# liruiluo/VLA-Adapter

Measured on AMD Instinct MI355X. Metric: fine-tune samples/sec (224px img + 32-tok prompt), adapter-only, fwd+bwd+AdamW, higher is better.
Workload: dtype bf16

## Files before the change

### vla_adapter_amd/csrc/gemm256.hip

```cpp
#include <type_traits>
#include "gemm_epilogue.h"
#include "gemm_params.h"

namespace {

constexpr int BK = 64;
constexpr int HT = 16384;
constexpr int LDS_BYTES = 8 * HT;
constexpr int STG = 8192;

#define VLA_MMA_QUADRANT(Q, FB, FA)                                                                                                   \
  do {                                                                                                                                \
    if constexpr (F8) {                                                                                                               \
      _Pragma("unroll") for (int ni = 0; ni < 2; ++ni)                                                                                \
        _Pragma("unroll") for (int mi = 0; mi < 4; ++mi)                                                                              \
          Q[ni][mi] = __builtin_amdgcn_mfma_scale_f32_16x16x128_f8f6f4(cat8(FB[ni][0], FB[ni][1]), cat8(FA[mi][0], FA[mi][1]), Q[ni][mi], \
                                                                       0, 0, 0, 0x7f7f7f7f, 0, 0x7f7f7f7f);                            \
    } else {                                                                                                                          \
      _Pragma("unroll") for (int s = 0; s < 2; ++s)                                                                                   \
        _Pragma("unroll") for (int ni = 0; ni < 2; ++ni)                                                                              \
          _Pragma("unroll") for (int mi = 0; mi < 4; ++mi)                                                                            \
            Q[ni][mi] = __builtin_amdgcn_mfma_f32_16x16x32_bf16(FB[ni][s], FA[mi][s], Q[ni][mi], 0, 0, 0);                            \
    }                                                                                                                                 \
  } while (0)

template <int EPI, bool F8 = false, bool RES = true, bool R2 = false, bool EXT = false>
__global__ __launch_bounds__(512) void gemm256_kernel(GemmP p) {
  extern __shared__ __attribute__((aligned(16))) char smem[];
  constexpr int EB = F8 ? 1 : 2;
  constexpr bool HAS_RES = EPI == 0 && RES;
  constexpr bool PRE = EPI != 2;
  const int tid = threadIdx.x, lane = tid & 63;
  const int wid = __builtin_amdgcn_readfirstlane(tid >> 6);
  const int wr = wid >> 2, wc = wid & 3;

  const int G = gridDim.x, bid = blockIdx.x;
  const int total = p.ntiles * p.batch;
  const int q8 = total >> 3, r8 = total & 7;
  const int xcd = bid & 7;
  auto rstart = [&](int x) { return x < r8 ? x * (q8 + 1) : r8 * (q8 + 1) + (x - r8) * q8; };
  int vt = bid;
  constexpr int GM = 6;
  int m0, n0, z;
  const char* Ab; const char* Bb;
  unsigned oa[2][2], ob[2][2];
  unsigned oa2[EXT ? 2 : 1][2], ob2[EXT ? 2 : 1][2];
  auto setup = [&](int swz) {
    int sl = lane;
    asm volatile("" : "+v"(sl));
    const int kc = ((sl & 7) ^ ((sl >> 3) & 7)) * 16;
    const int lrow = sl >> 3;
    int gA = p.gA;
    asm volatile("" : "+s"(gA));
    int ntl = p.ntiles;
    asm volatile("" : "+s"(ntl));
    z = swz / ntl;
    const int tl = swz - z * ntl;
    int br = ntl / p.tiles_n, bc = p.tiles_n;
    asm volatile("" : "+s"(br), "+s"(bc));
    const int pgb = GM * bc;
    const int grp = tl / pgb, rem = tl - grp * pgb;
    const int gmr = min(GM, br - grp * GM);
    m0 = (grp * GM + rem % gmr) * 256;
    n0 = (rem / gmr) * 256;
    Ab = reinterpret_cast<const char*>(p.A) + (long long)z * p.sA * EB;
    Bb = reinterpret_cast<const char*>(p.B) + (long long)z * p.sB * EB;
#pragma unroll
    for (int h = 0; h < 2; ++h)
#pragma unroll
      for (int j = 0; j < 2; ++j) {
        const int ra = min(m0 + wr * 128 + h * 64 + (wid & 3) * 16 + j * 8 + lrow, p.M - 1);
        oa[h][j] = (unsigned)(grouped_row(ra, gA, p.sgA, p.lda) * EB + kc);
        const int rb = min(n0 + (wid >> 1) * 64 + h * 32 + (wid & 1) * 16 + j * 8 + lrow, p.N - 1);
        ob[h][j] = (unsigned)((long long)rb * p.ldb * EB + kc);
        if constexpr (EXT) {
          oa2[h][j] = (unsigned)((long long)ra * p.lda2 * 2 + kc);
          ob2[h][j] = (unsigned)((long long)rb * p.ldb2 * 2 + kc);
        }
      }
  };
  const unsigned wdst = (unsigned)(size_t)((__attribute__((address_space(3))) char*)smem) + wid * 2048;
  auto stage_a = [&](int slot, int h, int k0) {
    if (EXT && k0 >= p.K) {
      const char* b2 = reinterpret_cast<const char*>(p.A2) + (k0 - p.K) * 2;
      glds16s(b2, oa2[EXT ? h : 0][0], wdst + slot * HT);
      glds16s(b2, oa2[EXT ? h : 0][1], wdst + slot * HT + 1024);
      return;
    }
    glds16s(Ab + k0 * 2, oa[h][0], wdst + slot * HT);
    glds16s(Ab + k0 * 2, oa[h][1], wdst + slot * HT + 1024);
  };
  auto stage_b = [&](int slot, int h, int k0) {
    if (EXT && k0 >= p.K) {
      const char* b2 = reinterpret_cast<const char*>(p.B2) + (k0 - p.K) * 2;
      glds16s(b2, ob2[EXT ? h : 0][0], wdst + slot * HT);
      glds16s(b2, ob2[EXT ? h : 0][1], wdst + slot * HT + 1024);
      return;
    }
    glds16s(Bb + k0 * 2, ob[h][0], wdst + slot * HT);
    glds16s(Bb + k0 * 2, ob[h][1], wdst + slot * HT + 1024);
  };
  auto stage_k0 = [&](int buf) {
    stage_b(buf * 4 + 0, 0, 0); stage_a(buf * 4 + 1, 0, 0); stage_b(buf * 4 + 2, 1, 0); stage_a(buf * 4 + 3, 1, 0);
  };
  uint2 braw[4];
  auto bias_vec = [&]() {
    const bf16_t* bias = (EPI != 2 && p.bias) ? p.bias + (long long)z * p.sBias : nullptr;
    return bias != nullptr && (((size_t)bias & 7) == 0) && p.N >= 4;
  };
  auto fetch_bias = [&](bool bvec) {
    int sl = lane;
    asm volatile("" : "+v"(sl));
    const int lq = sl >> 4;
    long long dist = bvec ? (long long)((uintptr_t)(p.bias + (long long)z * p.sBias) - (uintptr_t)p.B) : 0;
    int lim = bvec ? p.N : 0;
    asm volatile("" : "+s"(dist), "+s"(lim));
    const bf16_t* src = reinterpret_cast<const bf16_t*>(reinterpret_cast<const char*>(p.B) + dist);
#pragma unroll
    for (int t4 = 0; t4 < 4; ++t4) {
      const int n = n0 + wc * 64 + t4 * 16 + lq * 4;
      braw[t4] = *reinterpret_cast<const uint2*>(src + (n + 3 < lim ? n : 0));
    }
  };

  const int nt = p.K / (F8 ? 2 * BK : BK) + (EXT ? p.K2 / BK : 0);

  const int aoff = wr * 64 * 128, boff = wc * 32 * 128;

  int cur = rstart(xcd) + (bid >> 3);
  if (p.stagger > 0 && (total - 1 - bid) / G + 1 < (total + G - 1) / G) {
    for (int i = 0; i < p.stagger; ++i) __builtin_amdgcn_s_sleep(16);
  }
  setup(cur);
  stage_k0(0);
  int d = 0;

  for (;;) {
    vt += G;
    const int nxt = vt < total ? rstart(vt & 7) + (vt >> 3) : -1;
    asm volatile("" : "+s"(cur));
    setup(cur);
    const bool bvec = bias_vec();
    if (nt > 1) {
      const int sn = (d ^ 1) * 4;
      stage_b(sn + 0, 0, BK); stage_a(sn + 1, 0, BK); stage_b(sn + 2, 1, BK);
    }
    fetch_bias(bvec);
    if (nt > 1) asm volatile("s_waitcnt vmcnt(10)" ::: "memory");
    else asm volatile("s_waitcnt vmcnt(4)" ::: "memory");
    VLA_BARRIER();
    int fl = lane;
    asm volatile("" : "+v"(fl));
    const int fo0 = (fl & 15) * 128 + ((((F8 ? 2 * (fl >> 4) : 0 + (fl >> 4))) ^ (fl & 7)) << 4);
    const int fo1 = (fl & 15) * 128 + ((((F8 ? 2 * (fl >> 4) + 1 : 4 + (fl >> 4))) ^ (fl & 7)) << 4);
    if (wr == 1) VLA_BARRIER();

    f32x4 acc[2][2][2][4];
#pragma unroll
    for (int a = 0; a < 2; ++a)
#pragma unroll
      for (int b = 0; b < 2; ++b)
#pragma unroll
        for (int c = 0; c < 2; ++c)
#pragma unroll
          for (int e = 0; e < 4; ++e) acc[a][b][c][e] = f32x4{0.f, 0.f, 0.f, 0.f};

    bf16x8 fa[4][2], fb0[2][2], fb1[2][2];
    for (int t = 0; t < nt; ++t) {
      const char* kb = smem + d * 4 * HT;
      const int so = d * 4, sn = (d ^ 1) * 4;
      {
        const char* sb = kb + 0 * HT + boff;
#pragma unroll
        for (int ni = 0; ni < 2; ++ni) {
          fb0[ni][0] = *reinterpret_cast<const bf16x8*>(sb + ni * 2048 + fo0);
          fb0[ni][1] = *reinterpret_cast<const bf16x8*>(sb + ni * 2048 + fo1);
        }
        const char* sa = kb + 1 * HT + aoff;
#pragma unroll
        for (int mi = 0; mi < 4; ++mi) {
          fa[mi][0] = *reinterpret_cast<const bf16x8*>(sa + mi * 2048 + fo0);
          fa[mi][1] = *reinterpret_cast<const bf16x8*>(sa + mi * 2048 + fo1);
        }
        const char* sb1 = kb + 2 * HT + boff;
#pragma unroll
        for (int ni = 0; ni < 2; ++ni) {
          fb1[ni][0] = *reinterpret_cast<const bf16x8*>(sb1 + ni * 2048 + fo0);
          fb1[ni][1] = *reinterpret_cast<const bf16x8*>(sb1 + ni * 2048 + fo1);
        }
        __builtin_amdgcn_sched_barrier(0);
        if (t + 1 < nt) {
          stage_a(sn + 3, 1, (t + 1) * BK);
          if (t > 0) asm volatile("s_waitcnt vmcnt(8)" ::: "memory");
        } else if (t > 0) {
          asm volatile("s_waitcnt vmcnt(0)" ::: "memory");
        }
        asm volatile("s_waitcnt lgkmcnt(0)" ::: "memory");
        VLA_BARRIER();
        __builtin_amdgcn_s_setprio(1);
        VLA_MMA_QUADRANT(acc[0][0], fb0, fa);
        VLA_MMA_QUADRANT(acc[0][1], fb1, fa);
        __builtin_amdgcn_s_setprio(0);
        VLA_BARRIER();
      }
      {
        const char* sa = kb + 3 * HT + aoff;
#pragma unroll
        for (int mi = 0; mi < 4; ++mi) {
          fa[mi][0] = *reinterpret_cast<const bf16x8*>(sa + mi * 2048 + fo0);
          fa[mi][1] = *reinterpret_cast<const bf16x8*>(sa + mi * 2048 + fo1);
        }
        __builtin_amdgcn_sched_barrier(0);
        if (t + 2 < nt) {
          stage_b(so + 0, 0, (t + 2) * BK); stage_a(so + 1, 0, (t + 2) * BK); stage_b(so + 2, 1, (t + 2) * BK);
          asm volatile("s_waitcnt vmcnt(8)" ::: "memory");
        } else if (t + 1 < nt) {
          asm volatile("s_waitcnt vmcnt(2)" ::: "memory");
        } else {
          asm volatile("s_waitcnt vmcnt(0)" ::: "memory");
        }
        asm volatile("s_waitcnt lgkmcnt(0)" ::: "memory");
        VLA_BARRIER();
        __builtin_amdgcn_s_setprio(1);
        VLA_MMA_QUADRANT(acc[1][1], fb1, fa);
        VLA_MMA_QUADRANT(acc[1][0], fb0, fa);
        __builtin_amdgcn_s_setprio(0);
        VLA_BARRIER();
      }
      d ^= 1;
    }
    if (wr == 0) VLA_BARRIER();
    asm volatile("s_waitcnt lgkmcnt(0)" ::: "memory");

    const int em0 = m0, en0 = n0, ez = z;
    int el = lane;
    asm volatile("" : "+v"(el));
    const int lq = el >> 4, lr = el & 15;
    int gR = p.gR, gC = p.gC, res_mod = p.res_mod, c_live_mod = p.c_live_mod;
    asm volatile("" : "+s"(gR), "+s"(gC), "+s"(res_mod), "+s"(c_live_mod));
    const bf16_t* bias = (EPI != 2 && p.bias) ? p.bias + (long long)ez * p.sBias : nullptr;
    const int wn0 = en0 + wc * 64;
    if constexpr (F8) {
#pragma unroll
      for (int t4 = 0; t4 < 4; ++t4) {
        float sbv[4];
#pragma unroll
        for (int j = 0; j < 4; ++j) sbv[j] = p.scaleB[min(wn0 + t4 * 16 + lq * 4 + j, p.N - 1)];
#pragma unroll
        for (int mh = 0; mh < 2; ++mh)
#pragma unroll
          for (int mi = 0; mi < 4; ++mi) {
            const float sav = p.scaleA[min(em0 + wr * 128 + mh * 64 + mi * 16 + lr, p.M - 1)];
#pragma unroll
            for (int j = 0; j < 4; ++j) acc[mh][t4 >> 1][t4 & 1][mi][j] *= sav * sbv[j];
          }
      }
    }
    float bv[4][4];
    int ebvec = __builtin_amdgcn_readfirstlane(bias_vec() ? 1 : 0);
    asm volatile("" : "+s"(ebvec));
#pragma unroll
    for (int t4 = 0; t4 < 4; ++t4) {
      const int n = wn0 + t4 * 16 + lq * 4;
      const bool ok = ebvec != 0 && n + 3 < p.N;
      bv[t4][0] = ok ? bf_lo(braw[t4].x) : 0.f; bv[t4][1] = ok ? bf_hi(braw[t4].x) : 0.f;
      bv[t4][2] = ok ? bf_lo(braw[t4].y) : 0.f; bv[t4][3] = ok ? bf_hi(braw[t4].y) : 0.f;
      if (bias && !ok) {
#pragma unroll
        for (int j = 0; j < 4; ++j)
          if (n + j < p.N) bv[t4][j] = bf2f(bias[n + j]);
      }
    }
    bf16_t* Cb = p.C + (long long)ez * p.sC;
    const bf16_t* Rb = (HAS_RES && p.R) ? p.R + (long long)ez * p.sR : nullptr;
    const bool vec_ok = ((p.ldc & 7) == 0) && (!Rb || (p.ldr & 7) == 0);
    const bool plain_rows = (res_mod | gR | gC | c_live_mod) == 0;
    const bool live_rows = EPI == 1 && (res_mod | gR | gC) == 0 && c_live_mod >= 64;
    bool skip[2], inside[2], fastm[2];
#pragma unroll
    for (int mh = 0; mh < 2; ++mh) {
      const int wm0 = em0 + wr * 128 + mh * 64;
      skip[mh] = wm0 >= p.M || wn0 >= p.N;
      inside[mh] = wm0 + 64 <= p.M && wn0 + 64 <= p.N;
      fastm[mh] = EPI != 2 && (plain_rows || live_rows) && vec_ok && inside[mh] && !skip[mh];
    }
    u32x4 rv[2][8];
    int fres0 = 0, fres1 = 0;
    const char* rsrc = nullptr;
    if constexpr (HAS_RES) {
      long long rdist = Rb ? (long long)((uintptr_t)Rb - (uintptr_t)p.B) : 0;
      fres0 = __builtin_amdgcn_readfirstlane((fastm[0] && Rb) ? 1 : 0);
      fres1 = __builtin_amdgcn_readfirstlane((fastm[1] && Rb) ? 1 : 0);
      asm volatile("" : "+s"(rdist), "+s"(fres0), "+s"(fres1));
      rsrc = reinterpret_cast<const char*>(p.B) + rdist;
    }
    auto load_res = [&](int mh, int it0, int it1) {
#pragma unroll
      for (int it = it0; it < it1; ++it) {
        const long long off = ((long long)(em0 + wr * 128 + mh * 64 + it * 8 + (el >> 3)) * p.ldr + wn0 + (el & 7) * 8) * 2;
        rv[mh][it] = *reinterpret_cast<const u32x4*>(rsrc + ((mh == 0 ? fres0 : fres1) ? off : 0));
      }
    };
    auto drop_res = [&](int mh) {
      asm volatile("" ::"v"(rv[mh][0]), "v"(rv[mh][1]), "v"(rv[mh][2]), "v"(rv[mh][3]), "v"(rv[mh][4]), "v"(rv[mh][5]), "v"(rv[mh][6]),
                   "v"(rv[mh][7]));
    };
    if (PRE && nxt >= 0) { setup(nxt); stage_k0(d); }
    char* const reg = PRE ? smem + (d ^ 1) * 4 * HT + wid * STG : smem + wid * STG;
    if constexpr (HAS_RES) load_res(0, 0, 4);

    if constexpr (EPI == 2) {
#pragma unroll
      for (int mh = 0; mh < 2; ++mh) {
        const int wm0 = em0 + wr * 128 + mh * 64;
        auto A4 = [&](int t4, int mi) -> f32x4& { return acc[mh][t4 >> 1][t4 & 1][mi]; };
          const bf16_t* GU = p.R + (long long)ez * p.sR;
          bf16_t* Cb = p.C + (long long)ez * p.sC;
          constexpr int ROWB = 2 * 64 * 2 + 16;
          char* reg2 = smem + wid * (32 * ROWB);
#pragma unroll
          for (int half = 0; half < 2; ++half) {
#pragma unroll
            for (int mq = 0; mq < 2; ++mq) {
              const int mi = 2 * half + mq;
              const int m = min(wm0 + mi * 16 + lr, p.M - 1);
#pragma unroll
              for (int t4 = 0; t4 < 4; ++t4) {
                const int hc = wn0 + t4 * 16 + lq * 4;
                const long long go = grouped_row(m, gR, p.sgR, p.ldr) + (hc >> 4) * 32 + (hc & 15);
                const bool ok = hc + 3 < p.N;
                const uint2 gv = ok ? *reinterpret_cast<const uint2*>(GU + go) : uint2{0, 0};
                const uint2 uv = ok ? *reinterpret_cast<const uint2*>(GU + go + 16) : uint2{0, 0};
                float gg[4], uu[4], dg[4], du[4];
                unpack4(gv, gg);
                unpack4(uv, uu);
#pragma unroll
                for (int j = 0; j < 4; ++j) swiglu_bwd(rbf(A4(t4, mi)[j] * p.alpha), gg[j], uu[j], dg[j], du[j]);
                char* rowp = reg2 + (mq * 16 + lr) * ROWB + (t4 * 32 + lq * 4) * 2;
                *reinterpret_cast<uint2*>(rowp) = pack4(dg);
                *reinterpret_cast<uint2*>(rowp + 32) = pack4(du);
              }
            }
#pragma unroll
            for (int it = 0; it < 8; ++it) {
              const int row = it * 4 + (el >> 4), ch = el & 15;
              const int m = wm0 + half * 32 + row, n2 = 2 * wn0 + ch * 8;
              if (m < p.M && n2 + 8 <= 2 * p.N)
                *reinterpret_cast<uint4*>(Cb + (long long)m * p.ldc + n2) = *reinterpret_cast<const uint4*>(reg2 + row * ROWB + ch * 16);
            }
          }
      }
    } else {
      uint2 pk[2][4][4];
      uint2 hp[2][2][4];
      if constexpr (EPI == 1) {
        const bool plain = bias == nullptr && p.alpha == 1.f;
#pragma unroll
        for (int mh = 0; mh < 2; ++mh)
#pragma unroll
          for (int pr = 0; pr < 2; ++pr)
#pragma unroll
            for (int mi = 0; mi < 4; ++mi) {
              f32x4 ga = acc[mh][pr][0][mi], ua = acc[mh][pr][1][mi];
              if (!plain) {
#pragma unroll
                for (int j = 0; j < 4; ++j) { ga[j] = epi_linear(ga[j], p.alpha, bv[2 * pr][j]); ua[j] = epi_linear(ua[j], p.alpha, bv[2 * pr + 1][j]); }
              }
              const uint2 gp = pack4(ga), up = pack4(ua);
              float g[4], u[4], h[4];
              unpack4(gp, g);
              unpack4(up, u);
#pragma unroll
              for (int j = 0; j < 4; ++j) h[j] = swiglu_h(g[j], u[j]);
              pk[mh][2 * pr][mi] = gp;
              pk[mh][2 * pr + 1][mi] = up;
              hp[mh][pr][mi] = pack4(h);
            }
      } else {
        auto phase_a = [&](auto fn, auto post_t) {
          constexpr bool POST = decltype(post_t)::value;
          const float alpha = p.alpha;
#pragma unroll
          for (int mh = 0; mh < 2; ++mh)
#pragma unroll
            for (int t4 = 0; t4 < 4; ++t4)
#pragma unroll
              for (int mi = 0; mi < 4; ++mi) {
                const f32x4 a = acc[mh][t4 >> 1][t4 & 1][mi];
                float x[4];
#pragma unroll
                for (int j = 0; j < 4; ++j) {
                  x[j] = fn(epi_linear<POST>(a[j], alpha, bv[t4][j]));
                }
                pk[mh][t4][mi] = uint2{pack2(x[0], x[1]), pack2(x[2], x[3])};
              }
        };
        auto phase_a_rope = [&]() {
          const float alpha = p.alpha;
#pragma unroll
          for (int mh = 0; mh < 2; ++mh)
#pragma unroll
            for (int mi = 0; mi < 4; ++mi) {
              const int pos = min(em0 + wr * 128 + mh * 64 + mi * 16 + lr, p.M - 1) % p.rope_T;
#pragma unroll
              for (int ni = 0; ni < 2; ++ni) {
                const int d = ni * 16 + lq * 4;
                const f32x4 c = *reinterpret_cast<const f32x4*>(p.rope_cos + (long long)pos * 32 + d);
                const f32x4 sn = *reinterpret_cast<const f32x4*>(p.rope_sin + (long long)pos * 32 + d);
                const f32x4 xa = acc[mh][0][ni][mi], xb = acc[mh][1][ni][mi];
                float ya[4], yb[4];
#pragma unroll
                for (int j = 0; j < 4; ++j) {
                  const float a = rbf(epi_linear(xa[j], alpha, bv[ni][j])), b = rbf(epi_linear(xb[j], alpha, bv[ni + 2][j]));
                  ya[j] = rope_rot_a(a, b, c[j], sn[j]);
                  yb[j] = rope_rot_b(a, b, c[j], sn[j]);
                }
                pk[mh][ni][mi] = uint2{pack2(ya[0], ya[1]), pack2(ya[2], ya[3])};
                pk[mh][ni + 2][mi] = uint2{pack2(yb[0], yb[1]), pack2(yb[2], yb[3])};
              }
              __builtin_amdgcn_sched_barrier(0);
            }
        };
        auto phase_a_rope2 = [&](auto post_t) {
          constexpr bool POST = decltype(post_t)::value;
          const float alpha = p.alpha;
#pragma unroll
          for (int mh = 0; mh < 2; ++mh)
#pragma unroll
            for (int mi = 0; mi < 4; ++mi) {
              const int pos = min(em0 + wr * 128 + mh * 64 + mi * 16 + lr, p.M - 1) % p.rope_T;
#pragma unroll
              for (int t4 = 0; t4 < 4; ++t4) {
                const int d = (wn0 + t4 * 16 + lq * 4) % p.rope_dh;
                const f32x4 c = *reinterpret_cast<const f32x4*>(p.rope_cos + (long long)pos * p.rope_dh + d);
                const f32x4 sn = *reinterpret_cast<const f32x4*>(p.rope_sin + (long long)pos * p.rope_dh + d);
                const f32x4 a = acc[mh][t4 >> 1][t4 & 1][mi];
                float x[4];
#pragma unroll
                for (int j = 0; j < 4; ++j) {
                  x[j] = rbf(epi_linear<POST>(a[j], alpha, bv[t4][j]));
                }
                const float y0 = rope_rot_a(x[0], x[1], c[0], sn[0]), y1 = rope_rot_b(x[0], x[1], c[1], sn[1]);
                const float y2 = rope_rot_a(x[2], x[3], c[2], sn[2]), y3 = rope_rot_b(x[2], x[3], c[3], sn[3]);
                pk[mh][t4][mi] = uint2{pack2(y0, y1), pack2(y2, y3)};
                if (t4 & 1) __builtin_amdgcn_sched_barrier(0);
              }
            }
        };
        if (p.rope_mode == 1 && wn0 < p.rope_cols) phase_a_rope();
        else if (R2 && p.rope_mode == 2 && wn0 < p.rope_cols) {
          if (p.bias_post) phase_a_rope2(std::true_type{});
          else phase_a_rope2(std::false_type{});
        } else if (p.bias_post) phase_a(ActNone{}, std::true_type{});
        else if (p.act == VLA_ACT_GELU) phase_a(ActGelu{}, std::false_type{});
        else if (p.act == VLA_ACT_RELU) phase_a(ActRelu{}, std::false_type{});
        else if (p.act == VLA_ACT_GELU_TANH) phase_a(ActGeluTanh{}, std::false_type{});
        else phase_a(ActNone{}, std::false_type{});
      }
#pragma unroll
      for (int mh = 0; mh < 2; ++mh)
#pragma unroll
        for (int t4 = 0; t4 < 4; ++t4)
          asm volatile("" : "+v"(pk[mh][t4][0].x), "+v"(pk[mh][t4][0].y), "+v"(pk[mh][t4][1].x), "+v"(pk[mh][t4][1].y),
                            "+v"(pk[mh][t4][2].x), "+v"(pk[mh][t4][2].y), "+v"(pk[mh][t4][3].x), "+v"(pk[mh][t4][3].y));
      asm volatile("" : "+v"(el));
      if constexpr (HAS_RES) { load_res(0, 4, 8); load_res(1, 0, 8); }
#pragma unroll
      for (int mh = 0; mh < 2; ++mh) {
        const int wm0 = em0 + wr * 128 + mh * 64;
        if (skip[mh]) {
          if constexpr (HAS_RES) drop_res(mh);
          continue;
        }
        if constexpr (EPI == 1) {
          bf16_t* C2 = p.C2 + (long long)ez * p.sC2;
          constexpr int HSTR = 32 * 2 + 16;
#pragma unroll
          for (int pr = 0; pr < 2; ++pr)
#pragma unroll
            for (int mi = 0; mi < 4; ++mi)
              *reinterpret_cast<uint2*>(reg + (mi * 16 + lr) * HSTR + (pr * 16 + lq * 4) * 2) = hp[mh][pr][mi];
          const bool hvec = ((p.ldc2 & 7) == 0) && (((size_t)C2 & 15) == 0);
          uint4 hv[4];
#pragma unroll
          for (int it = 0; it < 4; ++it) hv[it] = *reinterpret_cast<const uint4*>(reg + (it * 16 + (el >> 2)) * HSTR + (el & 3) * 16);
          __builtin_amdgcn_sched_barrier(0);
#pragma unroll
          for (int it = 0; it < 4; ++it) {
            const int row = it * 16 + (el >> 2), ch = el & 3;
            const int m = wm0 + row, hc = (wn0 >> 1) + ch * 8;
            const uint4 v = hv[it];
            if (hvec && inside[mh]) {
              *reinterpret_cast<uint4*>(C2 + (long long)m * p.ldc2 + hc) = v;
              continue;
            }
            if (m >= p.M || hc >= (p.N >> 1)) continue;
            bf16_t* dst = C2 + (long long)m * p.ldc2 + hc;
            if (hvec && hc + 8 <= (p.N >> 1)) {
              *reinterpret_cast<uint4*>(dst) = v;
            } else {
              const unsigned wv[4] = {v.x, v.y, v.z, v.w};
#pragma unroll
              for (int k = 0; k < 8; ++k)
                if (hc + k < (p.N >> 1)) dst[k] = (bf16_t)((k & 1) ? (wv[k >> 1] >> 16) : (wv[k >> 1] & 0xffffu));
            }
          }
          if (p.C == nullptr) continue;
          if (c_live_mod > 0 && (wm0 % c_live_mod) + 63 < p.c_live_from) continue;
        }
#pragma unroll
        for (int t4 = 0; t4 < 4; ++t4)
#pragma unroll
          for (int mi = 0; mi < 4; ++mi) {
            const int row = mi * 16 + lr;
            *reinterpret_cast<uint2*>(reg + row * 128 + (((t4 * 2 + (lq >> 1)) ^ ((row >> 1) & 7)) << 4) + (lq & 1) * 8) = pk[mh][t4][mi];
          }
        if (fastm[mh]) {
          uint4 vv[8];
#pragma unroll
          for (int it = 0; it < 8; ++it) {
            const int row = it * 8 + (el >> 3), ch = el & 7;
            vv[it] = *reinterpret_cast<const uint4*>(reg + row * 128 + ((ch ^ ((row >> 1) & 7)) << 4));
          }
          __builtin_amdgcn_sched_barrier(0);
          auto store_fast = [&](auto live_t) {
          constexpr bool LIVE = decltype(live_t)::value;
          int lpos = 0;
          if constexpr (LIVE) lpos = __builtin_amdgcn_readfirstlane(wm0 % c_live_mod);
#pragma unroll
          for (int it = 0; it < 8; ++it) {
            const int row = it * 8 + (el >> 3), ch = el & 7;
            if constexpr (LIVE) {
              int pos = lpos + row;
              if (pos >= c_live_mod) pos -= c_live_mod;
              if (pos < p.c_live_from) continue;
            }
            uint4 v = vv[it];
            if constexpr (HAS_RES) {
              const u32x4 r = rv[mh][it];
              const unsigned a[4] = {v.x, v.y, v.z, v.w};
              unsigned o[4];
#pragma unroll
              for (int k = 0; k < 4; ++k) o[k] = (mh == 0 ? fres0 : fres1) ? add_packed2(a[k], r[k]) : a[k];
              v = uint4{o[0], o[1], o[2], o[3]};
            }
            *reinterpret_cast<uint4*>(Cb + (long long)(wm0 + row) * p.ldc + wn0 + ch * 8) = v;
          }
          };
          if (EPI == 1 && c_live_mod > 0) store_fast(std::true_type{});
          else store_fast(std::false_type{});
          continue;
        }
        auto store_rows = [&](auto fast_t) {
          constexpr bool FAST = decltype(fast_t)::value;
#pragma nounroll
          for (int it = 0; it < 8; ++it) {
            const int row = it * 8 + (el >> 3), ch = el & 7;
            const int m = wm0 + row, n = wn0 + ch * 8;
            uint4 v = *reinterpret_cast<const uint4*>(reg + row * 128 + ((ch ^ ((row >> 1) & 7)) << 4));
            if (m >= p.M || n >= p.N) continue;
            long long roff, crow;
            if constexpr (FAST) {
              roff = (long long)m * p.ldr;
              crow = (long long)m * p.ldc;
            } else {
              if (!row_live(m, c_live_mod, p.c_live_from)) continue;
              roff = residual_row(m, res_mod, gR, p.sgR, p.ldr);
              crow = grouped_row(m, gC, p.sgC, p.ldc);
            }
            if (vec_ok && n + 8 <= p.N) {
              if (Rb) v = add_packed8(v, *reinterpret_cast<const uint4*>(Rb + roff + n));
              *reinterpret_cast<uint4*>(Cb + crow + n) = v;
            } else {
              store_tail8(Cb, crow, Rb, roff, v, n, p.N);
            }
          }
        };
        if constexpr (HAS_RES) drop_res(mh);
        if (plain_rows) store_rows(std::true_type{});
        else store_rows(std::false_type{});
      }
    }

    if (nxt < 0) break;
    VLA_BARRIER();
    if (!PRE) { setup(nxt); stage_k0(d); }
    cur = nxt;
  }
}

int num_cus() {
  static int n = 0;
  if (n == 0) {
    int dev = 0;
    if (hipGetDevice(&dev) != hipSuccess || hipDeviceGetAttribute(&n, hipDeviceAttributeMultiprocessorCount, dev) != hipSuccess || n <= 0) n = 256;
  }
  return n;
}

template <int EPI, bool F8 = false, bool RES = true, bool R2 = false, bool EXT = false>
int launch256(const GemmP& p0, int batch, long long grid, hipStream_t st) {
  if (int rc = vla_lds_limit<gemm256_kernel<EPI, F8, RES, R2, EXT>>(LDS_BYTES, "gemm256_kernel")) return rc;
  GemmP p = p0;
  p.tiles_n = (p.N + 255) / 256;
  p.ntiles = ((p.M + 255) / 256) * p.tiles_n;
  p.batch = batch;
  const long long total = (long long)p.ntiles * batch;
  if (grid <= 0 || grid > total) grid = total;
  p.stagger = 0;
  if (total > grid && total % grid != 0) {
    const long long tile_cycles = (long long)((p.K + (EXT ? p.K2 : 0)) / BK) * 2128 + 13000;
    p.stagger = (int)(tile_cycles / 2 / 1024);
  }
  hipLaunchKernelGGL((gemm256_kernel<EPI, F8, RES, R2, EXT>), dim3((unsigned)grid), dim3(512), LDS_BYTES, st, p);
  return VLA_OK;
}

}

int vla_num_cus() { return num_cus(); }

int vla_gemm256_launch(const GemmP& p, int epi, int batch, long long grid, hipStream_t st) {
  if (p.K2 > 0) {
    if (epi == 1) return launch256<1, false, true, false, true>(p, 1, grid, st);
    return p.R ? launch256<0, false, true, false, true>(p, 1, grid, st) : launch256<0, false, false, false, true>(p, 1, grid, st);
  }
  if (p.scaleA != nullptr) return epi == 1 ? launch256<1, true>(p, batch, grid, st) : launch256<0, true>(p, batch, grid, st);
  if (p.rope_mode == 2) return launch256<0, false, false, true>(p, batch, grid, st);
  if (epi == 1) return launch256<1>(p, batch, grid, st);
  if (epi == 2) return launch256<2>(p, batch, grid, st);
  return p.R ? launch256<0, false, true>(p, batch, grid, st) : launch256<0, false, false>(p, batch, grid, st);
}
```

Before: 1326.

## Prefetch residual tile into LDS during final K iterations of last tile

On a workgroup's last output tile, when the residual is aligned and un-grouped, the kernel issues async global-to-LDS loads of the first half of the residual block during the last K-loop steps. The epilogue then reads those rows from LDS instead of from global memory after the MMA loop. This is meant to hide residual-load latency behind the final MMAs. It adds LDS reuse of the A/B staging buffers, new vmcnt bookkeeping and a templated epilogue branch, which raises code size and the chance of wait-count or buffer-overlap errors.

```diff
diff --git a/vla_adapter_amd/csrc/gemm256.hip b/vla_adapter_amd/csrc/gemm256.hip
--- a/vla_adapter_amd/csrc/gemm256.hip
+++ b/vla_adapter_amd/csrc/gemm256.hip
@@ -146,6 +146,26 @@
       stage_b(sn + 0, 0, BK); stage_a(sn + 1, 0, BK); stage_b(sn + 2, 1, BK);
     }
     fetch_bias(bvec);
+    int rpre = 0;
+    if constexpr (HAS_RES) {
+      const bf16_t* Rt = p.R ? p.R + (long long)z * p.sR : nullptr;
+      const bool ok = nxt < 0 && Rt != nullptr && (((size_t)Rt & 15) == 0) && ((p.ldc | p.ldr) & 7) == 0 &&
+                      (p.res_mod | p.gR | p.gC | p.c_live_mod) == 0 && m0 + wr * 128 + 64 <= p.M && n0 + wc * 64 + 64 <= p.N;
+      rpre = __builtin_amdgcn_readfirstlane(ok ? 1 : 0);
+    }
+    auto res_off = [&](int it) { return it < 6 ? wid * 6144 + it * 1024 : 3 * HT + wid * 2048 + (it - 6) * 1024; };
+    auto stage_res = [&](int buf, int i0, int i1) {
+      int sl = lane;
+      asm volatile("" : "+v"(sl));
+      int ldr = p.ldr;
+      asm volatile("" : "+s"(ldr));
+      const char* rb = reinterpret_cast<const char*>(p.R) + ((long long)z * p.sR + (long long)(m0 + wr * 128) * ldr + n0 + wc * 64) * 2;
+      const unsigned rowo = (unsigned)((sl >> 3) * ldr * 2);
+      const unsigned dst = (unsigned)(size_t)((__attribute__((address_space(3))) char*)smem) + buf * 4 * HT;
+#pragma unroll
+      for (int it = i0; it < i1; ++it)
+        glds16s(rb + (long long)it * 8 * ldr * 2, rowo + ((unsigned)((sl & 7) ^ ((it * 4 + (sl >> 4)) & 7)) << 4), dst + res_off(it));
+    };
     if (nt > 1) asm volatile("s_waitcnt vmcnt(10)" ::: "memory");
     else asm volatile("s_waitcnt vmcnt(4)" ::: "memory");
     VLA_BARRIER();
@@ -192,6 +212,13 @@
         if (t + 1 < nt) {
           stage_a(sn + 3, 1, (t + 1) * BK);
           if (t > 0) asm volatile("s_waitcnt vmcnt(8)" ::: "memory");
+        } else if (HAS_RES && rpre) {
+          if (t > 0) {
+            stage_res(d ^ 1, 6, 8);
+            asm volatile("s_waitcnt vmcnt(8)" ::: "memory");
+          } else {
+            stage_res(d ^ 1, 0, 8);
+          }
         } else if (t > 0) {
           asm volatile("s_waitcnt vmcnt(0)" ::: "memory");
         }
@@ -215,8 +242,13 @@
           stage_b(so + 0, 0, (t + 2) * BK); stage_a(so + 1, 0, (t + 2) * BK); stage_b(so + 2, 1, (t + 2) * BK);
           asm volatile("s_waitcnt vmcnt(8)" ::: "memory");
         } else if (t + 1 < nt) {
-          asm volatile("s_waitcnt vmcnt(2)" ::: "memory");
-        } else {
+          if (HAS_RES && rpre) {
+            stage_res(d, 0, 6);
+            asm volatile("s_waitcnt vmcnt(8)" ::: "memory");
+          } else {
+            asm volatile("s_waitcnt vmcnt(2)" ::: "memory");
+          }
+        } else if (!(HAS_RES && rpre)) {
           asm volatile("s_waitcnt vmcnt(0)" ::: "memory");
         }
         asm volatile("s_waitcnt lgkmcnt(0)" ::: "memory");
@@ -284,7 +316,7 @@
       inside[mh] = wm0 + 64 <= p.M && wn0 + 64 <= p.N;
       fastm[mh] = EPI != 2 && (plain_rows || live_rows) && vec_ok && inside[mh] && !skip[mh];
     }
-    u32x4 rv[2][8];
+    u32x4 re[4];
     int fres0 = 0, fres1 = 0;
     const char* rsrc = nullptr;
     if constexpr (HAS_RES) {
@@ -294,20 +326,17 @@
       asm volatile("" : "+s"(rdist), "+s"(fres0), "+s"(fres1));
       rsrc = reinterpret_cast<const char*>(p.B) + rdist;
     }
-    auto load_res = [&](int mh, int it0, int it1) {
-#pragma unroll
-      for (int it = it0; it < it1; ++it) {
-        const long long off = ((long long)(em0 + wr * 128 + mh * 64 + it * 8 + (el >> 3)) * p.ldr + wn0 + (el & 7) * 8) * 2;
-        rv[mh][it] = *reinterpret_cast<const u32x4*>(rsrc + ((mh == 0 ? fres0 : fres1) ? off : 0));
-      }
-    };
-    auto drop_res = [&](int mh) {
-      asm volatile("" ::"v"(rv[mh][0]), "v"(rv[mh][1]), "v"(rv[mh][2]), "v"(rv[mh][3]), "v"(rv[mh][4]), "v"(rv[mh][5]), "v"(rv[mh][6]),
-                   "v"(rv[mh][7]));
+    auto res_at = [&](int mh, int it) {
+      return ((long long)(em0 + wr * 128 + mh * 64 + it * 8 + (el >> 3)) * p.ldr + wn0 + (el & 7) * 8) * 2;
     };
     if (PRE && nxt >= 0) { setup(nxt); stage_k0(d); }
     char* const reg = PRE ? smem + (d ^ 1) * 4 * HT + wid * STG : smem + wid * STG;
-    if constexpr (HAS_RES) load_res(0, 0, 4);
+    if constexpr (HAS_RES) {
+      if (rpre) asm volatile("s_waitcnt vmcnt(0)" ::: "memory");
+      const int mhe = rpre, frese = rpre ? fres1 : fres0;
+#pragma unroll
+      for (int it = 0; it < 4; ++it) re[it] = *reinterpret_cast<const u32x4*>(rsrc + (frese ? res_at(mhe, it) : 0));
+    }
 
     if constexpr (EPI == 2) {
 #pragma unroll
@@ -464,7 +493,24 @@
           asm volatile("" : "+v"(pk[mh][t4][0].x), "+v"(pk[mh][t4][0].y), "+v"(pk[mh][t4][1].x), "+v"(pk[mh][t4][1].y),
                             "+v"(pk[mh][t4][2].x), "+v"(pk[mh][t4][2].y), "+v"(pk[mh][t4][3].x), "+v"(pk[mh][t4][3].y));
       asm volatile("" : "+v"(el));
-      if constexpr (HAS_RES) { load_res(0, 4, 8); load_res(1, 0, 8); }
+      auto phase_b = [&](auto pre_t) {
+      constexpr bool LPRE = decltype(pre_t)::value;
+      u32x4 rv[2][8];
+      auto load_res = [&](int mh, int it0, int it1) {
+#pragma unroll
+        for (int it = it0; it < it1; ++it)
+          rv[mh][it] = *reinterpret_cast<const u32x4*>(rsrc + ((mh == 0 ? fres0 : fres1) ? res_at(mh, it) : 0));
+      };
+      auto drop_res = [&](int mh) {
+        asm volatile("" ::"v"(rv[mh][0]), "v"(rv[mh][1]), "v"(rv[mh][2]), "v"(rv[mh][3]), "v"(rv[mh][4]), "v"(rv[mh][5]), "v"(rv[mh][6]),
+                     "v"(rv[mh][7]));
+      };
+      if constexpr (HAS_RES) {
+#pragma unroll
+        for (int it = 0; it < 4; ++it) rv[LPRE ? 1 : 0][it] = re[it];
+        if constexpr (LPRE) load_res(1, 4, 8);
+        else { load_res(0, 4, 8); load_res(1, 0, 8); }
+      }
 #pragma unroll
       for (int mh = 0; mh < 2; ++mh) {
         const int wm0 = em0 + wr * 128 + mh * 64;
@@ -521,6 +567,16 @@
           for (int it = 0; it < 8; ++it) {
             const int row = it * 8 + (el >> 3), ch = el & 7;
             vv[it] = *reinterpret_cast<const uint4*>(reg + row * 128 + ((ch ^ ((row >> 1) & 7)) << 4));
+          }
+          if constexpr (LPRE) {
+            if (mh == 0) {
+              const char* rl = smem + d * 4 * HT;
+#pragma unroll
+              for (int it = 0; it < 8; ++it) {
+                const int row = it * 8 + (el >> 3), ch = el & 7;
+                rv[0][it] = *reinterpret_cast<const u32x4*>(rl + res_off(it) + (el >> 3) * 128 + ((ch ^ ((row >> 1) & 7)) << 4));
+              }
+            }
           }
           __builtin_amdgcn_sched_barrier(0);
           auto store_fast = [&](auto live_t) {
@@ -579,6 +635,13 @@
         if constexpr (HAS_RES) drop_res(mh);
         if (plain_rows) store_rows(std::true_type{});
         else store_rows(std::false_type{});
+      }
+      };
+      if constexpr (HAS_RES) {
+        if (rpre) phase_b(std::true_type{});
+        else phase_b(std::false_type{});
+      } else {
+        phase_b(std::false_type{});
       }
     }
 
```

Result: no change. 1323 (-0.2%).
